# adalca/neurite

Measured on AMD Instinct MI355X. Metric: Mvoxels/sec interpn+Dice on 160^3 x 32-label, higher is better.
Workload: dtype f32

## Files before the change

neurite_amd/csrc/fused_wc.h:

```cpp

#pragma once

#include <type_traits>

#include "dice_reduce.h"
#include "interpn_core.h"

namespace {

#ifndef WC_NST_WARP
#define WC_NST_WARP 3
#endif
#ifndef WC_NST_FUSED
#define WC_NST_FUSED 2
#endif
#ifndef WC_NST_BWD
#define WC_NST_BWD 3
#endif
constexpr int WC_SLOTS = 128;
constexpr int WC_OVF = 16;
constexpr int WC_TRASH_ROW = WC_SLOTS + WC_OVF;
constexpr int WC_ROWS = WC_TRASH_ROW + 1;
constexpr unsigned WC_NOROW = 0x01ffffffu;
constexpr unsigned WC_TAGS_OFF = WC_ROWS * 128;
constexpr unsigned WC_LIST_OFF = WC_TAGS_OFF + 528;
constexpr unsigned WC_BC_OFF = WC_LIST_OFF + 512;
constexpr unsigned WC_WAVE_BYTES = WC_BC_OFF + 128;
constexpr unsigned WC_BLOCK_BYTES = 4 * WC_WAVE_BYTES;
static_assert(WC_LIST_OFF % 16 == 0 && WC_BC_OFF % 16 == 0 && WC_WAVE_BYTES % 16 == 0, "LDS layout");
static_assert((WC_SLOTS + 1) * 4 <= 528 && WC_ROWS <= 256, "LDS layout");
static_assert(2 * WC_BLOCK_BYTES <= 160 * 1024, "two blocks per CU");

typedef __attribute__((address_space(3))) char wc_lds_char;
typedef __attribute__((address_space(3))) nrt_f4 wc_lds_f4;
typedef __attribute__((address_space(3))) volatile nrt_i4 wc_lds_vi4;
typedef __attribute__((address_space(3))) volatile unsigned wc_lds_vu32;
typedef unsigned wc_u3 __attribute__((ext_vector_type(3)));
typedef unsigned wc_u4 __attribute__((ext_vector_type(4)));
typedef float wc_f3 __attribute__((ext_vector_type(3)));

__device__ __forceinline__ void wc_corner(float pv, float mx, int &i0, int &i1, float &w0) {
    const float cl = fminf(fmaxf(pv, 0.0f), mx);
    const float l0 = floorf(cl);
    const float l1 = fminf(nrt_add(l0, 1.0f), mx);
    i0 = (int)l0; i1 = (int)l1;
    w0 = nrt_sub(l1, cl);
}

__device__ __forceinline__ __amdgpu_buffer_rsrc_t wc_rsrc(const void *base, unsigned bytes) {
    const unsigned long long v = (unsigned long long)base;
    const void *u = (const void *)(((unsigned long long)(unsigned)__builtin_amdgcn_readfirstlane((unsigned)(v >> 32)) << 32) |
                                   (unsigned long long)(unsigned)__builtin_amdgcn_readfirstlane((unsigned)v));
    return __builtin_amdgcn_make_buffer_rsrc((void *)u, 0, __builtin_amdgcn_readfirstlane((int)bytes), 0x00020000);
}

struct WcBwd {
    const float *sums, *gdice;
    float eps;
    float *gloc;
};

template <int MODE, bool STORE, bool MM, bool FILL, bool DICE, int BWD = 0>
__device__ __forceinline__ void wc_item(const InterpArgs &a, const TileGeom &tg, const float *__restrict__ fixed, float *__restrict__ fpart,
                                        float *__restrict__ mpart, const XmWork &xw, char *wc_smem, const WcBwd &bw = WcBwd{nullptr, nullptr, 0.0f, nullptr}) {
    constexpr int G = 8, L = 32;
    static_assert(BWD == 0 || (DICE && !STORE && !MM), "the backward form reads a second row per voxel and stores the location gradient only");
    const int b = __builtin_amdgcn_readfirstlane(xw.b);
    const unsigned prow = (unsigned)__builtin_amdgcn_readfirstlane((int)xw.prow), ucol = (unsigned)__builtin_amdgcn_readfirstlane((int)xw.ucol);
    const unsigned RY = 1u << tg.lry, RZ = 1u << tg.lrz;
    const unsigned nRz = (tg.nTz + RZ - 1) / RZ;
    const unsigned reg = ucol / (RY * RZ), wr = ucol % (RY * RZ);
    const unsigned cy = (reg / nRz) * RY + wr / RZ, cz = (reg % nRz) * RZ + wr % RZ;
    const int x0 = __builtin_amdgcn_readfirstlane(xw.x0), y0 = (int)cy << 2, z0 = (int)cz << 3;
    int npass = __builtin_amdgcn_readfirstlane(xw.xlen);
    if (cy >= tg.nTy || cz >= tg.nTz || npass < 0) npass = 0;

    const int lane = threadIdx.x & 63, wave = threadIdx.x >> 6;
    const int g = lane >> 3, p = lane & 7;
    const int dzt = (0x1320 >> ((g & 3) * 4)) & 15;
    const int yy = y0 + 2 * (wave >> 1) + (g >> 2), zz = z0 + 4 * (wave & 1) + dzt;
    const bool yzvalid = (yy < a.O[1]) && (zz < a.O[2]);
    const int yc = min(yy, a.O[1] - 1), zc = min(zz, a.O[2] - 1);
    const unsigned qyz = (unsigned)yc * (unsigned)a.O[2] + (unsigned)zc, qstep = (unsigned)a.O[1] * (unsigned)a.O[2];
    const unsigned SY = (unsigned)a.S[1], SZ = (unsigned)a.S[2];
    const float mxx = (float)(a.S[0] - 1), mxy = (float)(a.S[1] - 1), mxz = (float)(a.S[2] - 1);
    const float fyc = (float)yc, fzc = (float)zc;
    const float ly = (yc == 0) ? 0.0f : ((yc == a.O[1] - 1) ? mxy : nrt_mul(a.delta[1], fyc));
    const float lz = (zc == 0) ? 0.0f : ((zc == a.O[2] - 1) ? mxz : nrt_mul(a.delta[2], fzc));

    const char *volb = (const char *)a.vol + (long long)b * a.vol_bs * 4ll;
    const unsigned long long volbytes = (unsigned long long)a.S[0] * SY * SZ * 128ull;
    const unsigned outbytes = a.nout * 128u;
    const __amdgpu_buffer_rsrc_t vres = wc_rsrc(volb, (unsigned)volbytes);
    const __amdgpu_buffer_rsrc_t lres = wc_rsrc(MODE != NRT_LOC_LINSPACE ? (const char *)(a.loc + (long long)b * a.loc_bs) : volb, a.nout * 12u);
    const __amdgpu_buffer_rsrc_t fres = wc_rsrc(DICE ? (const char *)fixed + (long long)b * a.out_bs * 4ll : volb, outbytes);
    const __amdgpu_buffer_rsrc_t ores = wc_rsrc(STORE ? (const char *)a.out + (long long)b * a.out_bs * 4ll : volb, outbytes);
    const __amdgpu_buffer_rsrc_t gres = wc_rsrc(BWD ? (const char *)(bw.gloc + (long long)b * a.nout * 3) : volb, a.nout * 12u);
    const unsigned gl_lane = (p == 0 && yzvalid) ? qyz * 12u : 0xffffffffu;
    float ca[4] = {0.0f, 0.0f, 0.0f, 0.0f}, cb[4] = {0.0f, 0.0f, 0.0f, 0.0f};
    if (BWD == 1) {
        const float *sm = bw.sums + (long long)b * 3 * L;
#pragma unroll
        for (int k = 0; k < 4; ++k) {
            const int l = p * 4 + k;
            const float num = 2.0f * sm[l] + bw.eps, den = sm[L + l] + sm[2 * L + l] + bw.eps;
            const float gd = bw.gdice[(long long)b * L + l];
            if (den != 0.0f) { ca[k] = 2.0f * gd / den; cb[k] = -2.0f * gd * num / (den * den); }
        }
    }
    const unsigned loc_lane = qyz * 12u, row_lane = (qyz * 8u + (unsigned)p) * 16u;
    const unsigned out_lane = yzvalid ? row_lane : 0xffffffffu;
    const unsigned loc_step = qstep * 12u, row_step = qstep * 128u;
    const unsigned p16 = (unsigned)p * 16u;

    wc_lds_char *wl = (wc_lds_char *)wc_smem + wave * WC_WAVE_BYTES;
    wc_lds_vu32 *tags = (wc_lds_vu32 *)(wl + WC_TAGS_OFF);
    wc_lds_char *lrow = wl + p * 16;
    tags[lane] = ~0u;
    tags[lane + 64] = ~0u;
    const bool cx1 = (p & 4) != 0, cy1 = (p & 2) != 0, cz1 = (p & 1) != 0;

    nrt_f2 stp_l = {0, 0}, stp_h = {0, 0}, stt_l = {0, 0}, stt_h = {0, 0}, spp_l = {0, 0}, spp_h = {0, 0};
    float mnt = INFINITY, mxt = -INFINITY, mnp = INFINITY, mxp = -INFINITY;

    struct Pass {
        float w0x, w0y, w0z;
        unsigned sl[8];
        unsigned lr[4], ld[4];
        unsigned xr[4], xd[4];
        int n;
        int xq;
        float mk[3];
        bool oob;
        nrt_f4 T;
        nrt_f4 F[4], Fx[4];
        float pn[3];
    };
    struct Mg { float w0x, w0y, w0z; bool oob, miss; unsigned rid, slot, t1, t2, mytag; float mk[3]; };
    constexpr int NST = ((BWD ? WC_NST_BWD : (DICE ? WC_NST_FUSED : WC_NST_WARP)) > 2) ? 3 : 2;
    constexpr bool XSH = NST == 3 && DICE;
    Pass A, B, C;
    nrt_f4 FxS[4] = {{0.f, 0.f, 0.f, 0.f}, {0.f, 0.f, 0.f, 0.f}, {0.f, 0.f, 0.f, 0.f}, {0.f, 0.f, 0.f, 0.f}};
    auto reset = [&](Pass &s) {
        s.w0x = s.w0y = s.w0z = 0.f; s.n = 0; s.xq = x0; s.oob = false; s.mk[0] = s.mk[1] = s.mk[2] = 0.f;
        s.T = (nrt_f4){0.f, 0.f, 0.f, 0.f};
#pragma unroll
        for (int i = 0; i < 4; ++i) { s.F[i] = s.Fx[i] = (nrt_f4){0.f, 0.f, 0.f, 0.f}; s.lr[i] = s.xr[i] = WC_NOROW << 7; s.ld[i] = s.xd[i] = WC_TRASH_ROW * 128u; }
#pragma unroll
        for (int i = 0; i < 8; ++i) s.sl[i] = 0;
        s.pn[0] = s.pn[1] = s.pn[2] = 0.f;
    };
    reset(A); reset(B);
    if (NST == 3) reset(C);

    auto fetch_loc = [&](int pass, Pass &s) {
        if (MODE != NRT_LOC_LINSPACE) {
            const wc_u3 v = __builtin_bit_cast(wc_u3, __builtin_amdgcn_raw_buffer_load_b96(lres, loc_lane, (unsigned)(x0 + pass) * loc_step, 0));
            s.pn[0] = __uint_as_float(v[0]); s.pn[1] = __uint_as_float(v[1]); s.pn[2] = __uint_as_float(v[2]);
        }
    };
    auto fetch_row = [&](unsigned rowoff) -> nrt_f4 {
        return __builtin_bit_cast(nrt_f4, __builtin_amdgcn_raw_buffer_load_b128(vres, rowoff | p16, 0, 0));
    };

    auto m1a = [&](int pass, const Pass &s, Mg &m) {
        const int xq = x0 + pass;
        float px, py, pz;
        if (MODE == NRT_LOC_ABSOLUTE) { px = s.pn[0]; py = s.pn[1]; pz = s.pn[2]; }
        else if (MODE == NRT_LOC_SHIFT) { px = nrt_add((float)xq, s.pn[0]); py = nrt_add(fyc, s.pn[1]); pz = nrt_add(fzc, s.pn[2]); }
        else { px = (xq == 0) ? 0.0f : ((xq == a.O[0] - 1) ? mxx : nrt_mul(a.delta[0], (float)xq)); py = ly; pz = lz; }
        int i0x, i1x, i0y, i1y, i0z, i1z;
        wc_corner(px, mxx, i0x, i1x, m.w0x);
        wc_corner(py, mxy, i0y, i1y, m.w0y);
        wc_corner(pz, mxz, i0z, i1z, m.w0z);
        m.oob = FILL ? ((px < 0.0f) || (px > mxx) || (py < 0.0f) || (py > mxy) || (pz < 0.0f) || (pz > mxz)) : false;
        if (BWD) {
            m.mk[0] = (fminf(fmaxf(px, 0.0f), mxx) == px) ? 1.0f : 0.0f;
            m.mk[1] = (fminf(fmaxf(py, 0.0f), mxy) == py) ? 1.0f : 0.0f;
            m.mk[2] = (fminf(fmaxf(pz, 0.0f), mxz) == pz) ? 1.0f : 0.0f;
        }
        const unsigned ix = cx1 ? i1x : i0x, iy = cy1 ? i1y : i0y, iz = cz1 ? i1z : i0z;
        m.rid = nrt_mad24(nrt_mad24(ix, SY, iy), SZ, iz);
        m.slot = ((ix & 3u) << 5) | ((iy & 3u) << 3) | (iz & 7u);
        m.mytag = (m.rid << 6) | (unsigned)lane;
        m.t1 = tags[m.slot];
    };
    auto m1b = [&](Mg &m) {
        m.miss = (m.t1 ^ m.mytag) >= 64u;
        tags[m.miss ? m.slot : (unsigned)WC_SLOTS] = m.mytag;
        m.t2 = tags[m.slot];
    };
    auto m1c = [&](int pass, const Mg &m, Pass &s) {
        const unsigned x2 = m.t2 ^ m.mytag;
        const bool served = x2 < 64u;
        const bool loader = m.miss && x2 == 0u;
        const bool orphan = !served;
        const unsigned long long Ml = __builtin_amdgcn_ballot_w64(loader), Mo = __builtin_amdgcn_ballot_w64(orphan);
        const unsigned long long Mf = Ml | Mo;
        const int no = __builtin_popcountll(Mo);
        int n = __builtin_popcountll(Mf);
        const unsigned ro = __builtin_amdgcn_mbcnt_hi((unsigned)(Mo >> 32), __builtin_amdgcn_mbcnt_lo((unsigned)Mo, 0u));
        const unsigned rf = __builtin_amdgcn_mbcnt_hi((unsigned)(Mf >> 32), __builtin_amdgcn_mbcnt_lo((unsigned)Mf, 0u));
        bool fetcher = loader || orphan;
        unsigned src = orphan ? (unsigned)WC_SLOTS + ro : m.slot;
        unsigned e = fetcher ? rf : (unsigned)n + ((unsigned)lane - rf);
        if (__builtin_expect(no > WC_OVF, 0)) {
            tags[lane] = ~0u;
            tags[lane + 64] = ~0u;
            e = (unsigned)lane; fetcher = true; src = (unsigned)lane; n = 64;
        }
        const unsigned src128 = src * 128u;
        const unsigned tp = ((e & 7u) << 3) | (e >> 3);
        typedef unsigned wc_u2 __attribute__((ext_vector_type(2)));
        *(__attribute__((address_space(3))) volatile wc_u2 *)(wl + WC_LIST_OFF + tp * 8u) =
            (wc_u2){fetcher ? (m.rid << 7) : (WC_NOROW << 7), fetcher ? src128 : (unsigned)WC_TRASH_ROW * 128u};
        ((__attribute__((address_space(3))) volatile unsigned short *)(wl + WC_BC_OFF))[lane] = (unsigned short)src128;
        const nrt_i4 la = *(wc_lds_vi4 *)(wl + WC_LIST_OFF + g * 64), lb = *(wc_lds_vi4 *)(wl + WC_LIST_OFF + g * 64 + 16);
        const nrt_i4 sh = *(wc_lds_vi4 *)(wl + WC_BC_OFF + g * 16);
        s.lr[0] = (unsigned)la[0]; s.ld[0] = (unsigned)la[1]; s.lr[1] = (unsigned)la[2]; s.ld[1] = (unsigned)la[3];
        s.lr[2] = (unsigned)lb[0]; s.ld[2] = (unsigned)lb[1]; s.lr[3] = (unsigned)lb[2]; s.ld[3] = (unsigned)lb[3];
        if (__builtin_expect(n > 32, 0)) {
            const nrt_i4 lc = *(wc_lds_vi4 *)(wl + WC_LIST_OFF + g * 64 + 32), le = *(wc_lds_vi4 *)(wl + WC_LIST_OFF + g * 64 + 48);
            s.xr[0] = (unsigned)lc[0]; s.xd[0] = (unsigned)lc[1]; s.xr[1] = (unsigned)lc[2]; s.xd[1] = (unsigned)lc[3];
            s.xr[2] = (unsigned)le[0]; s.xd[2] = (unsigned)le[1]; s.xr[3] = (unsigned)le[2]; s.xd[3] = (unsigned)le[3];
        }
#pragma unroll
        for (int c = 0; c < 4; ++c) { s.sl[2 * c] = (unsigned)sh[c] & 0xffffu; s.sl[2 * c + 1] = (unsigned)sh[c] >> 16; }
        s.w0x = m.w0x; s.w0y = m.w0y; s.w0z = m.w0z; s.oob = m.oob; s.n = n;
        if (BWD) { s.mk[0] = m.mk[0]; s.mk[1] = m.mk[1]; s.mk[2] = m.mk[2]; }
        s.xq = x0 + pass;
    };
    auto issue = [&](Pass &s) {
#pragma unroll
        for (int i = 0; i < 4; ++i) s.F[i] = fetch_row(s.lr[i]);
        if (!XSH && __builtin_expect(s.n > 32, 0)) {
#pragma unroll
            for (int i = 0; i < 4; ++i) s.Fx[i] = fetch_row(s.xr[i]);
        }
        if (DICE) s.T = __builtin_bit_cast(nrt_f4, __builtin_amdgcn_raw_buffer_load_b128(fres, row_lane, (unsigned)s.xq * row_step, 2));
    };
    auto issue_x = [&](Pass &s) {
        if (XSH && __builtin_expect(s.n > 32, 0)) {
#pragma unroll
            for (int i = 0; i < 4; ++i) FxS[i] = fetch_row(s.xr[i]);
        }
    };
    auto deliver = [&](Pass &s) {
#pragma unroll
        for (int i = 0; i < 4; ++i) *(wc_lds_f4 *)(lrow + s.ld[i]) = s.F[i];
        if (__builtin_expect(s.n > 32, 0)) {
#pragma unroll
            for (int i = 0; i < 4; ++i) *(wc_lds_f4 *)(lrow + s.xd[i]) = XSH ? FxS[i] : s.Fx[i];
        }
    };

    const int last = npass - 1;
    auto step = [&](int pass, Pass &s, Pass &o, Pass &nx, auto masked) {
        constexpr bool MASKED = decltype(masked)::value;
        issue(o);
        __builtin_amdgcn_sched_barrier(0);
        deliver(s);
        nrt_f4 R[8];
#pragma unroll
        for (int corner = 0; corner < 8; ++corner) R[corner] = *(const wc_lds_f4 *)(lrow + s.sl[corner]);
        __builtin_amdgcn_sched_barrier(0);
        Mg m;
        m1a(min(pass + NST, last), s, m);
        __builtin_amdgcn_sched_barrier(0);
        const float w1x = nrt_sub(1.0f, s.w0x), w1y = nrt_sub(1.0f, s.w0y), w1z = nrt_sub(1.0f, s.w0z);
        const nrt_f2 wy2 = {s.w0y, w1y}, wz2 = {s.w0z, w1z};
        const nrt_f2 wxy0 = (nrt_f2){s.w0x, s.w0x} * wy2, wxy1 = (nrt_f2){w1x, w1x} * wy2;
        nrt_f2 wt2[4];
        wt2[0] = (nrt_f2){wxy0[0], wxy0[0]} * wz2;
        wt2[1] = (nrt_f2){wxy0[1], wxy0[1]} * wz2;
        wt2[2] = (nrt_f2){wxy1[0], wxy1[0]} * wz2;
        wt2[3] = (nrt_f2){wxy1[1], wxy1[1]} * wz2;
        nrt_f2 al = {0.0f, 0.0f}, ah = {0.0f, 0.0f};
        constexpr bool BLEND = BWD != 2;
#pragma unroll
        for (int corner = 0; corner < (BLEND ? 4 : 0); ++corner) {
            const float wt = wt2[corner >> 1][corner & 1];
            const nrt_f2 w2 = {wt, wt};
            al = al + w2 * (nrt_f2){R[corner][0], R[corner][1]};
            ah = ah + w2 * (nrt_f2){R[corner][2], R[corner][3]};
        }
        asm volatile("" : "+v"(al), "+v"(ah));
        __builtin_amdgcn_sched_barrier(0);
        m1b(m);
        __builtin_amdgcn_sched_barrier(0);
#pragma unroll
        for (int corner = 4; corner < (BLEND ? 8 : 4); ++corner) {
            const float wt = wt2[corner >> 1][corner & 1];
            const nrt_f2 w2 = {wt, wt};
            al = al + w2 * (nrt_f2){R[corner][0], R[corner][1]};
            ah = ah + w2 * (nrt_f2){R[corner][2], R[corner][3]};
        }
        nrt_f4 acc = {al[0], al[1], ah[0], ah[1]};
        const unsigned xqcur = (unsigned)s.xq;
        const float cw0x = s.w0x, cw0y = s.w0y, cw0z = s.w0z, cmx = s.mk[0], cmy = s.mk[1], cmz = s.mk[2];
        const bool coob = s.oob;
        if (!BWD) {
            if (FILL) {
#pragma unroll
                for (int c = 0; c < 4; ++c) acc[c] = apply_fill(acc[c], s.oob, a.fill_f);
            }
            if (STORE) __builtin_amdgcn_raw_buffer_store_b128(__builtin_bit_cast(wc_u4, acc), ores, out_lane, (unsigned)s.xq * row_step, 2);
        }
        const nrt_f4 Tcur = s.T;
        asm volatile("" : "+v"(acc));
        __builtin_amdgcn_sched_barrier(0);
        m1c(min(pass + NST, last), m, s);
        __builtin_amdgcn_sched_barrier(0);
        if (BWD) {
            nrt_f2 gl2 = {Tcur[0], Tcur[1]}, gh2 = {Tcur[2], Tcur[3]};
            if (BWD == 1) {
                gl2 = __builtin_elementwise_fma((nrt_f2){cb[0], cb[1]}, (nrt_f2){acc[0], acc[1]}, (nrt_f2){ca[0], ca[1]} * gl2);
                gh2 = __builtin_elementwise_fma((nrt_f2){cb[2], cb[3]}, (nrt_f2){acc[2], acc[3]}, (nrt_f2){ca[2], ca[3]} * gh2);
            }
            if (FILL && coob) { gl2 = (nrt_f2){0.0f, 0.0f}; gh2 = gl2; }
            float gacc[3];
            loc_grad_rows(R, gl2, gh2, cw0x, w1x, cw0y, w1y, cw0z, w1z, cmx, cmy, cmz, gacc);
#pragma unroll
            for (int d = 0; d < 3; ++d) {
                float r = gacc[d];
                r += __int_as_float(__builtin_amdgcn_update_dpp(0, __float_as_int(r), 0xB1, 0xF, 0xF, true));
                r += __int_as_float(__builtin_amdgcn_update_dpp(0, __float_as_int(r), 0x4E, 0xF, 0xF, true));
                r += __int_as_float(__builtin_amdgcn_update_dpp(0, __float_as_int(r), 0x141, 0xF, 0xF, true));
                gacc[d] = r;
            }
            __builtin_amdgcn_raw_buffer_store_b96(__builtin_bit_cast(wc_u3, (wc_f3){gacc[0], gacc[1], gacc[2]}), gres, gl_lane, xqcur * loc_step, 0);
        } else if (DICE) {
            nrt_f4 T = Tcur;
            if (MASKED) {
#pragma unroll
                for (int c = 0; c < 4; ++c) { T[c] = yzvalid ? T[c] : 0.0f; acc[c] = yzvalid ? acc[c] : 0.0f; }
            }
            const nrt_f2 pl = {acc[0], acc[1]}, ph = {acc[2], acc[3]}, tl = {T[0], T[1]}, th = {T[2], T[3]};
            stp_l = stp_l + tl * pl; stp_h = stp_h + th * ph;
            stt_l = stt_l + tl * tl; stt_h = stt_h + th * th;
            spp_l = spp_l + pl * pl; spp_h = spp_h + ph * ph;
            if (MM) {
                if (!MASKED || yzvalid) {
#pragma unroll
                    for (int c = 0; c < 4; ++c) {
                        mnt = fminf(mnt, Tcur[c]); mxt = fmaxf(mxt, Tcur[c]);
                        mnp = fminf(mnp, acc[c]); mxp = fmaxf(mxp, acc[c]);
                    }
                }
            }
        }
        if (DICE && !BWD) asm volatile("" : "+v"(stp_l), "+v"(stp_h), "+v"(stt_l), "+v"(stt_h), "+v"(spp_l), "+v"(spp_h));
        else asm volatile("" :: "v"(acc));
        __builtin_amdgcn_sched_barrier(0);
        fetch_loc(min(pass + 2 * NST, last), s);
        issue_x(nx);
        __builtin_amdgcn_sched_barrier(0);
    };
    auto march = [&](auto masked) {
        Mg m;
        if constexpr (NST == 3) {
            fetch_loc(0, A);
            fetch_loc(min(1, last), B);
            fetch_loc(min(2, last), C);
            m1a(0, A, m); m1b(m); m1c(0, m, A);
            issue(A);
            fetch_loc(min(3, last), A);
            m1a(min(1, last), B, m); m1b(m); m1c(min(1, last), m, B);
            issue(B);
            fetch_loc(min(4, last), B);
            m1a(min(2, last), C, m); m1b(m); m1c(min(2, last), m, C);
            fetch_loc(min(5, last), C);
            issue_x(A);
            __builtin_amdgcn_sched_barrier(0);
            int pass = 0;
            for (; pass + 2 < npass; pass += 3) {
                step(pass, A, C, B, masked);
                step(pass + 1, B, A, C, masked);
                step(pass + 2, C, B, A, masked);
            }
            if (pass < npass) step(pass, A, C, B, masked);
            if (pass + 1 < npass) step(pass + 1, B, A, C, masked);
            return;
        }
        fetch_loc(0, A);
        fetch_loc(min(1, last), B);
        m1a(0, A, m); m1b(m); m1c(0, m, A);
        issue(A);
        fetch_loc(min(2, last), A);
        m1a(min(1, last), B, m); m1b(m); m1c(min(1, last), m, B);
        fetch_loc(min(3, last), B);
        __builtin_amdgcn_sched_barrier(0);
        int pass = 0;
        for (; pass + 1 < npass; pass += 2) {
            step(pass, A, B, B, masked);
            step(pass + 1, B, A, A, masked);
        }
        if (pass < npass) step(pass, A, B, B, masked);
    };
    if (npass > 0) {
        if (DICE && !BWD && __builtin_amdgcn_ballot_w64(!yzvalid) != 0ull) march(std::true_type());
        else march(std::false_type());
    }

    if (!DICE || BWD) return;
    nrt_f4 stp = {stp_l[0], stp_l[1], stp_h[0], stp_h[1]}, stt = {stt_l[0], stt_l[1], stt_h[0], stt_h[1]},
           spp = {spp_l[0], spp_l[1], spp_h[0], spp_h[1]};
#pragma unroll
    for (int c = 0; c < 4; ++c) {
        stp[c] = wave_xor_add(stp[c], G);
        stt[c] = wave_xor_add(stt[c], G);
        spp[c] = wave_xor_add(spp[c], G);
    }
    for (int off = 1; off < NRT_WAVE; off <<= 1) {
        mnt = fminf(mnt, __shfl_xor(mnt, off, NRT_WAVE)); mxt = fmaxf(mxt, __shfl_xor(mxt, off, NRT_WAVE));
        mnp = fminf(mnp, __shfl_xor(mnp, off, NRT_WAVE)); mxp = fmaxf(mxp, __shfl_xor(mxp, off, NRT_WAVE));
    }
    __syncthreads();
    float (*red)[3 * L + 4] = (float (*)[3 * L + 4])wc_smem;
    if (lane < G) {
#pragma unroll
        for (int c = 0; c < 4; ++c) {
            red[wave][0 * L + 4 * lane + c] = stp[c];
            red[wave][1 * L + 4 * lane + c] = stt[c];
            red[wave][2 * L + 4 * lane + c] = spp[c];
        }
    }
    if (lane == 0) { red[wave][3 * L + 0] = mnt; red[wave][3 * L + 1] = mxt; red[wave][3 * L + 2] = mnp; red[wave][3 * L + 3] = mxp; }
    __syncthreads();
    const long long pbase = (long long)b * tg.prows + prow;
    for (int i = threadIdx.x; i < 3 * L; i += 256) {
        float s = red[0][i];
#pragma unroll
        for (int w2 = 1; w2 < 4; ++w2) s += red[w2][i];
        fpart[pbase * 3 * L + i] = s;
    }
    if (threadIdx.x < 4) {
        float m = red[0][3 * L + threadIdx.x];
        for (int w2 = 1; w2 < 4; ++w2)
            m = (threadIdx.x & 1) ? fmaxf(m, red[w2][3 * L + threadIdx.x]) : fminf(m, red[w2][3 * L + threadIdx.x]);
        mpart[pbase * 4 + threadIdx.x] = m;
    }
    xmarch_zero_rows(tg, xw, 3 * L, fpart, mpart);
}


template <typename ITEM>
__device__ __forceinline__ void wc_persistent_loop(const TileGeom &tg, int O0, unsigned *__restrict__ queue, ITEM item) {
    __shared__ unsigned s_next[2];
    const unsigned home = blockIdx.x % NRT_NXCD;
    for (;;) {
        __syncthreads();
        if (threadIdx.x == 0) {
            unsigned kk = home, jb = 0xffffffffu;
            for (unsigned t = 0; t < NRT_NXCD; ++t) {
                const unsigned q = (home + t) % NRT_NXCD;
                const unsigned v = atomicAdd(&queue[q * 16u], 1u);
                if (v < tg.items_x) { kk = q; jb = v; break; }
            }
            s_next[0] = kk; s_next[1] = jb;
        }
        __syncthreads();
        const unsigned kk = s_next[0], jb = s_next[1];
        if (jb == 0xffffffffu) break;
        XmWork xw;
        if (!xmarch_work_at(tg, O0, kk, jb, xw)) continue;
        item(xw);
    }
    if (threadIdx.x == 0 && atomicAdd(&queue[NRT_NXCD * 16u], 1u) == gridDim.x - 1) {
        for (unsigned q = 0; q <= NRT_NXCD; ++q) queue[q * 16u] = 0u;
    }
}

template <int MODE, bool STORE, bool MM, bool FILL, bool DICE = true, bool PERSIST = false>
__global__ __launch_bounds__(256, 2) void warp_dice_wc(InterpArgs a, TileGeom tg, const float *__restrict__ fixed,
                                                        float *__restrict__ fpart, float *__restrict__ mpart, unsigned *__restrict__ queue) {
    extern __shared__ __attribute__((aligned(16))) char wc_smem[];
    if (!PERSIST) {
        XmWork xw;
        if (!xmarch_work(tg, a.O[0], xw)) return;
        wc_item<MODE, STORE, MM, FILL, DICE>(a, tg, fixed, fpart, mpart, xw, wc_smem);
        return;
    }
    wc_persistent_loop(tg, a.O[0], queue, [&](const XmWork &xw) { wc_item<MODE, STORE, MM, FILL, DICE>(a, tg, fixed, fpart, mpart, xw, wc_smem); });
}

template <int MODE, bool FILL, int BWD, bool PERSIST>
__global__ __launch_bounds__(256, 2) void warp_dice_wc_bwd(InterpArgs a, TileGeom tg, const float *__restrict__ rows, WcBwd bw,
                                                            unsigned *__restrict__ queue) {
    extern __shared__ __attribute__((aligned(16))) char wc_smem[];
    if (!PERSIST) {
        XmWork xw;
        if (!xmarch_work(tg, a.O[0], xw)) return;
        wc_item<MODE, false, false, FILL, true, BWD>(a, tg, rows, nullptr, nullptr, xw, wc_smem, bw);
        return;
    }
    wc_persistent_loop(tg, a.O[0], queue, [&](const XmWork &xw) { wc_item<MODE, false, false, FILL, true, BWD>(a, tg, rows, nullptr, nullptr, xw, wc_smem, bw); });
}

inline bool wc_persistent(const TileGeom &tg) { return NRT_NXCD * tg.items_x > 2u * (unsigned)nrt_num_cus(); }
static_assert(NRT_RING_GATHER_OFF == 0 && (NRT_NXCD + 1) * 16 <= NRT_RING_CCE_OFF, "the work counters of a launch stay in the gather's words of a slot");

template <int MODE, bool STORE, bool MM, bool FILL>
int launch_wc_inst(const InterpArgs &a, const TileGeom &tg, unsigned nblocks, int batch, const float *fixed, float *fpart, float *mpart,
                   hipStream_t st) {
    const unsigned items = NRT_NXCD * tg.items_x, slots = 2u * (unsigned)nrt_num_cus();
    unsigned *queue = wc_persistent(tg) ? nrt_ring_slot(st) : nullptr;
    if (queue) {
        if (hipFuncSetAttribute((const void *)warp_dice_wc<MODE, STORE, MM, FILL, true, true>, hipFuncAttributeMaxDynamicSharedMemorySize,
                                (int)WC_BLOCK_BYTES) != hipSuccess)
            return NRT_ERR_LAUNCH;
        hipLaunchKernelGGL((warp_dice_wc<MODE, STORE, MM, FILL, true, true>), dim3(nrt_xcd_grid(slots)), dim3(256), WC_BLOCK_BYTES, st, a, tg, fixed,
                           fpart, mpart, queue);
        return NRT_OK;
    }
    if (hipFuncSetAttribute((const void *)warp_dice_wc<MODE, STORE, MM, FILL>, hipFuncAttributeMaxDynamicSharedMemorySize, (int)WC_BLOCK_BYTES) != hipSuccess)
        return NRT_ERR_LAUNCH;
    hipLaunchKernelGGL((warp_dice_wc<MODE, STORE, MM, FILL>), dim3(items), dim3(256), WC_BLOCK_BYTES, st, a, tg, fixed, fpart, mpart,
                       (unsigned *)nullptr);
    (void)nblocks; (void)batch;
    return NRT_OK;
}

template <int MODE, bool FILL>
int launch_wc_fill(const InterpArgs &a, const TileGeom &tg, unsigned nblocks, int batch, bool store, bool minmax, const float *fixed,
                   float *fpart, float *mpart, hipStream_t st) {
    if (store) return minmax ? launch_wc_inst<MODE, true, true, FILL>(a, tg, nblocks, batch, fixed, fpart, mpart, st)
                             : launch_wc_inst<MODE, true, false, FILL>(a, tg, nblocks, batch, fixed, fpart, mpart, st);
    return minmax ? launch_wc_inst<MODE, false, true, FILL>(a, tg, nblocks, batch, fixed, fpart, mpart, st)
                  : launch_wc_inst<MODE, false, false, FILL>(a, tg, nblocks, batch, fixed, fpart, mpart, st);
}

template <int MODE>
int launch_wc_mode(const InterpArgs &a, const TileGeom &tg, unsigned nblocks, int batch, bool store, bool minmax, const float *fixed,
                   float *fpart, float *mpart, hipStream_t st) {
    return a.has_fill ? launch_wc_fill<MODE, true>(a, tg, nblocks, batch, store, minmax, fixed, fpart, mpart, st)
                      : launch_wc_fill<MODE, false>(a, tg, nblocks, batch, store, minmax, fixed, fpart, mpart, st);
}

inline bool wc_applies(const TileGeom &tg, int G, const InterpArgs &a) {
    return tg.x_march && G == 8 && tg.lty == 2 && tg.ltz == 3 && !tg.plane_major &&
           (unsigned long long)a.S[0] * a.S[1] * a.S[2] * 128ull < 0xffffff00ull;
}

inline int launch_wc(const InterpArgs &a, const TileGeom &tg, unsigned nblocks, int batch, int mode, bool store, bool minmax,
                     const float *fixed, float *fpart, float *mpart, hipStream_t st) {
    switch (mode) {
        case NRT_LOC_ABSOLUTE: return launch_wc_mode<NRT_LOC_ABSOLUTE>(a, tg, nblocks, batch, store, minmax, fixed, fpart, mpart, st);
        case NRT_LOC_SHIFT: return launch_wc_mode<NRT_LOC_SHIFT>(a, tg, nblocks, batch, store, minmax, fixed, fpart, mpart, st);
        default: return launch_wc_mode<NRT_LOC_LINSPACE>(a, tg, nblocks, batch, store, minmax, fixed, fpart, mpart, st);
    }
}

template <int MODE, bool FILL>
int launch_wc_interpn_inst(const InterpArgs &a, const TileGeom &tg, hipStream_t st) {
    const unsigned items = NRT_NXCD * tg.items_x, slots = 2u * (unsigned)nrt_num_cus();
    unsigned *queue = (items > slots) ? nrt_ring_slot(st) : nullptr;
    if (queue) {
        if (hipFuncSetAttribute((const void *)warp_dice_wc<MODE, true, false, FILL, false, true>, hipFuncAttributeMaxDynamicSharedMemorySize,
                                (int)WC_BLOCK_BYTES) != hipSuccess)
            return NRT_ERR_LAUNCH;
        hipLaunchKernelGGL((warp_dice_wc<MODE, true, false, FILL, false, true>), dim3(nrt_xcd_grid(slots)), dim3(256), WC_BLOCK_BYTES, st, a, tg,
                           (const float *)nullptr, (float *)nullptr, (float *)nullptr, queue);
        return NRT_OK;
    }
    if (hipFuncSetAttribute((const void *)warp_dice_wc<MODE, true, false, FILL, false>, hipFuncAttributeMaxDynamicSharedMemorySize,
                            (int)WC_BLOCK_BYTES) != hipSuccess)
        return NRT_ERR_LAUNCH;
    hipLaunchKernelGGL((warp_dice_wc<MODE, true, false, FILL, false>), dim3(items), dim3(256), WC_BLOCK_BYTES, st, a, tg, (const float *)nullptr,
                       (float *)nullptr, (float *)nullptr, (unsigned *)nullptr);
    return NRT_OK;
}

template <int MODE, bool FILL, int BWD>
int launch_wc_bwd_inst(const InterpArgs &a, const TileGeom &tg, const float *rows, const WcBwd &bw, hipStream_t st) {
    const unsigned items = NRT_NXCD * tg.items_x, slots = 2u * (unsigned)nrt_num_cus();
    unsigned *queue = (items > slots) ? nrt_ring_slot(st) : nullptr;
    if (queue) {
        if (hipFuncSetAttribute((const void *)warp_dice_wc_bwd<MODE, FILL, BWD, true>, hipFuncAttributeMaxDynamicSharedMemorySize, (int)WC_BLOCK_BYTES) != hipSuccess)
            return NRT_ERR_LAUNCH;
        hipLaunchKernelGGL((warp_dice_wc_bwd<MODE, FILL, BWD, true>), dim3(nrt_xcd_grid(slots)), dim3(256), WC_BLOCK_BYTES, st, a, tg, rows, bw, queue);
        return NRT_OK;
    }
    if (hipFuncSetAttribute((const void *)warp_dice_wc_bwd<MODE, FILL, BWD, false>, hipFuncAttributeMaxDynamicSharedMemorySize, (int)WC_BLOCK_BYTES) != hipSuccess)
        return NRT_ERR_LAUNCH;
    hipLaunchKernelGGL((warp_dice_wc_bwd<MODE, FILL, BWD, false>), dim3(items), dim3(256), WC_BLOCK_BYTES, st, a, tg, rows, bw, (unsigned *)nullptr);
    return NRT_OK;
}

template <int MODE, bool FILL>
int launch_wc_bwd_mode(const InterpArgs &a, const TileGeom &tg, const float *rows, const WcBwd &bw, hipStream_t st) {
    return bw.sums ? launch_wc_bwd_inst<MODE, FILL, 1>(a, tg, rows, bw, st) : launch_wc_bwd_inst<MODE, FILL, 2>(a, tg, rows, bw, st);
}

}

int nrt_wc_bwd_launch(const void *args, int batch, int mode, const float *rows, const float *sums, const float *grad_dice, float eps,
                      float *grad_loc, void *stream) {
    const InterpArgs &a = *(const InterpArgs *)args;
    if (mode != NRT_LOC_ABSOLUTE && mode != NRT_LOC_SHIFT) return NRT_ERR_INVALID_ARG;
    TileGeom tg;
    unsigned nblocks, grid;
    const int t = xmarch_default_tune();
    tile_geometry(a.O, 8, t, t, tg, nblocks);
    xmarch_setup_mixed(a.O, batch, t, tg, grid);
    hipStream_t st = nrt_stream(stream);
    const WcBwd bw = {sums, grad_dice, eps, grad_loc};
    int rc;
    if (mode == NRT_LOC_ABSOLUTE) rc = a.has_fill ? launch_wc_bwd_mode<NRT_LOC_ABSOLUTE, true>(a, tg, rows, bw, st) : launch_wc_bwd_mode<NRT_LOC_ABSOLUTE, false>(a, tg, rows, bw, st);
    else rc = a.has_fill ? launch_wc_bwd_mode<NRT_LOC_SHIFT, true>(a, tg, rows, bw, st) : launch_wc_bwd_mode<NRT_LOC_SHIFT, false>(a, tg, rows, bw, st);
    if (rc != NRT_OK) return rc;
    NRT_CHECK_LAUNCH();
    return NRT_OK;
}

bool nrt_wc_interpn_supported(const void *args, int batch) {
    const InterpArgs &a = *(const InterpArgs *)args;
    if (a.C != 32 || !xmarch_applies(a.O, batch)) return false;
    if ((unsigned long long)a.nout * 128ull >= (1ull << 32)) return false;
    if ((long long)a.S[0] * a.S[1] >= (1 << 24) || a.S[2] >= (1 << 24) || (long long)a.O[0] * a.O[1] >= (1 << 24) || a.O[2] >= (1 << 24)) return false;
    TileGeom tg;
    unsigned nblocks, grid;
    const int t = xmarch_default_tune();
    tile_geometry(a.O, 8, t, t, tg, nblocks);
    xmarch_setup_mixed(a.O, batch, t, tg, grid);
    return wc_applies(tg, 8, a);
}

int nrt_wc_interpn_launch(const void *args, int batch, int mode, void *stream) {
    const InterpArgs &a = *(const InterpArgs *)args;
    TileGeom tg;
    unsigned nblocks, grid;
    const int t = xmarch_default_tune();
    tile_geometry(a.O, 8, t, t, tg, nblocks);
    xmarch_setup_mixed(a.O, batch, t, tg, grid);
    hipStream_t st = nrt_stream(stream);
    int rc;
    switch (mode) {
        case NRT_LOC_ABSOLUTE: rc = a.has_fill ? launch_wc_interpn_inst<NRT_LOC_ABSOLUTE, true>(a, tg, st) : launch_wc_interpn_inst<NRT_LOC_ABSOLUTE, false>(a, tg, st); break;
        case NRT_LOC_SHIFT: rc = a.has_fill ? launch_wc_interpn_inst<NRT_LOC_SHIFT, true>(a, tg, st) : launch_wc_interpn_inst<NRT_LOC_SHIFT, false>(a, tg, st); break;
        default: rc = a.has_fill ? launch_wc_interpn_inst<NRT_LOC_LINSPACE, true>(a, tg, st) : launch_wc_interpn_inst<NRT_LOC_LINSPACE, false>(a, tg, st); break;
    }
    if (rc != NRT_OK) return rc;
    NRT_CHECK_LAUNCH();
    return NRT_OK;
}
```

Measured before the change: 19810.

## Batch sample geometry across passes through per-wave LDS records

```diff
diff --git a/neurite_amd/csrc/fused_wc.h b/neurite_amd/csrc/fused_wc.h
--- a/neurite_amd/csrc/fused_wc.h
+++ b/neurite_amd/csrc/fused_wc.h
@@ -25,11 +25,14 @@
 constexpr unsigned WC_TAGS_OFF = WC_ROWS * 128;
 constexpr unsigned WC_LIST_OFF = WC_TAGS_OFF + 528;
 constexpr unsigned WC_BC_OFF = WC_LIST_OFF + 512;
-constexpr unsigned WC_WAVE_BYTES = WC_BC_OFF + 128;
+constexpr unsigned WC_REC_OFF = WC_BC_OFF + 128;
+constexpr unsigned WC_REC_GROUP = 80;
+constexpr unsigned WC_WAVE_BYTES = WC_REC_OFF + 8 * WC_REC_GROUP;
 constexpr unsigned WC_BLOCK_BYTES = 4 * WC_WAVE_BYTES;
-static_assert(WC_LIST_OFF % 16 == 0 && WC_BC_OFF % 16 == 0 && WC_WAVE_BYTES % 16 == 0, "LDS layout");
+static_assert(WC_LIST_OFF % 16 == 0 && WC_BC_OFF % 16 == 0 && WC_REC_OFF % 16 == 0 && WC_WAVE_BYTES % 16 == 0, "LDS layout");
 static_assert((WC_SLOTS + 1) * 4 <= 528 && WC_ROWS <= 256, "LDS layout");
 static_assert(2 * WC_BLOCK_BYTES <= 160 * 1024, "two blocks per CU");
+static_assert(2 * (WC_BLOCK_BYTES + 8) <= 160 * 1024, "two blocks per CU, the work item's words of a persistent block included");
 
 typedef __attribute__((address_space(3))) char wc_lds_char;
 typedef __attribute__((address_space(3))) nrt_f4 wc_lds_f4;
@@ -45,6 +48,12 @@
     const float l1 = fminf(nrt_add(l0, 1.0f), mx);
     i0 = (int)l0; i1 = (int)l1;
     w0 = nrt_sub(l1, cl);
+}
+
+__device__ __forceinline__ unsigned wc_mad24_su(unsigned a, unsigned b_uniform, unsigned c) {
+    unsigned r;
+    asm("v_mad_u32_u24 %0, %1, %2, %3" : "=v"(r) : "v"(a), "s"(b_uniform), "v"(c));
+    return r;
 }
 
 __device__ __forceinline__ __amdgpu_buffer_rsrc_t wc_rsrc(const void *base, unsigned bytes) {
@@ -134,7 +143,6 @@
         bool oob;
         nrt_f4 T;
         nrt_f4 F[4], Fx[4];
-        float pn[3];
     };
     struct Mg { float w0x, w0y, w0z; bool oob, miss; unsigned rid, slot, t1, t2, mytag; float mk[3]; };
     constexpr int NST = ((BWD ? WC_NST_BWD : (DICE ? WC_NST_FUSED : WC_NST_WARP)) > 2) ? 3 : 2;
@@ -148,40 +156,69 @@
         for (int i = 0; i < 4; ++i) { s.F[i] = s.Fx[i] = (nrt_f4){0.f, 0.f, 0.f, 0.f}; s.lr[i] = s.xr[i] = WC_NOROW << 7; s.ld[i] = s.xd[i] = WC_TRASH_ROW * 128u; }
 #pragma unroll
         for (int i = 0; i < 8; ++i) s.sl[i] = 0;
-        s.pn[0] = s.pn[1] = s.pn[2] = 0.f;
     };
     reset(A); reset(B);
     if (NST == 3) reset(C);
 
-    auto fetch_loc = [&](int pass, Pass &s) {
-        if (MODE != NRT_LOC_LINSPACE) {
-            const wc_u3 v = __builtin_bit_cast(wc_u3, __builtin_amdgcn_raw_buffer_load_b96(lres, loc_lane, (unsigned)(x0 + pass) * loc_step, 0));
-            s.pn[0] = __uint_as_float(v[0]); s.pn[1] = __uint_as_float(v[1]); s.pn[2] = __uint_as_float(v[2]);
-        }
-    };
     auto fetch_row = [&](unsigned rowoff) -> nrt_f4 {
         return __builtin_bit_cast(nrt_f4, __builtin_amdgcn_raw_buffer_load_b128(vres, rowoff | p16, 0, 0));
     };
 
-    auto m1a = [&](int pass, const Pass &s, Mg &m) {
-        const int xq = x0 + pass;
+    constexpr int PER = NST == 2 ? 4 : 3;
+    static_assert(PER * 20 <= WC_REC_GROUP && WC_REC_GROUP % 16 == 0 && PER % NST == 0, "geometry batches");
+    const int last = npass - 1;
+    const int pj = p % PER;
+    wc_lds_char *rec_rd = wl + WC_REC_OFF + g * WC_REC_GROUP;
+    float bl[3] = {0.f, 0.f, 0.f};
+    auto batch_fetch = [&](int kb) {
+        if (MODE != NRT_LOC_LINSPACE) {
+            const unsigned xq = (unsigned)(x0 + min(kb * PER + pj, last));
+            const wc_u3 v = __builtin_bit_cast(wc_u3, __builtin_amdgcn_raw_buffer_load_b96(lres, loc_lane + xq * loc_step, 0, 0));
+            bl[0] = __uint_as_float(v[0]); bl[1] = __uint_as_float(v[1]); bl[2] = __uint_as_float(v[2]);
+        }
+    };
+    auto batch_compute = [&](int kb) {
+        const int xq = x0 + min(kb * PER + pj, last);
         float px, py, pz;
-        if (MODE == NRT_LOC_ABSOLUTE) { px = s.pn[0]; py = s.pn[1]; pz = s.pn[2]; }
-        else if (MODE == NRT_LOC_SHIFT) { px = nrt_add((float)xq, s.pn[0]); py = nrt_add(fyc, s.pn[1]); pz = nrt_add(fzc, s.pn[2]); }
+        if (MODE == NRT_LOC_ABSOLUTE) { px = bl[0]; py = bl[1]; pz = bl[2]; }
+        else if (MODE == NRT_LOC_SHIFT) { px = nrt_add((float)xq, bl[0]); py = nrt_add(fyc, bl[1]); pz = nrt_add(fzc, bl[2]); }
         else { px = (xq == 0) ? 0.0f : ((xq == a.O[0] - 1) ? mxx : nrt_mul(a.delta[0], (float)xq)); py = ly; pz = lz; }
         int i0x, i1x, i0y, i1y, i0z, i1z;
-        wc_corner(px, mxx, i0x, i1x, m.w0x);
-        wc_corner(py, mxy, i0y, i1y, m.w0y);
-        wc_corner(pz, mxz, i0z, i1z, m.w0z);
-        m.oob = FILL ? ((px < 0.0f) || (px > mxx) || (py < 0.0f) || (py > mxy) || (pz < 0.0f) || (pz > mxz)) : false;
+        float w0x, w0y, w0z;
+        wc_corner(px, mxx, i0x, i1x, w0x);
+        wc_corner(py, mxy, i0y, i1y, w0y);
+        wc_corner(pz, mxz, i0z, i1z, w0z);
+        const bool oob = FILL ? ((px < 0.0f) || (px > mxx) || (py < 0.0f) || (py > mxy) || (pz < 0.0f) || (pz > mxz)) : false;
+        unsigned w2 = (((unsigned)i1x & 3u) << 5) | (((unsigned)i1y & 3u) << 3) | ((unsigned)i1z & 7u);
+        w2 |= ((unsigned)(i1x - i0x) << 8) | ((unsigned)(i1y - i0y) << 16) | ((unsigned)(i1z - i0z) << 24) | (oob ? 1u << 25 : 0u);
         if (BWD) {
-            m.mk[0] = (fminf(fmaxf(px, 0.0f), mxx) == px) ? 1.0f : 0.0f;
-            m.mk[1] = (fminf(fmaxf(py, 0.0f), mxy) == py) ? 1.0f : 0.0f;
-            m.mk[2] = (fminf(fmaxf(pz, 0.0f), mxz) == pz) ? 1.0f : 0.0f;
-        }
-        const unsigned ix = cx1 ? i1x : i0x, iy = cy1 ? i1y : i0y, iz = cz1 ? i1z : i0z;
-        m.rid = nrt_mad24(nrt_mad24(ix, SY, iy), SZ, iz);
-        m.slot = ((ix & 3u) << 5) | ((iy & 3u) << 3) | (iz & 7u);
+            w2 |= (fminf(fmaxf(px, 0.0f), mxx) == px) ? 1u << 26 : 0u;
+            w2 |= (fminf(fmaxf(py, 0.0f), mxy) == py) ? 1u << 27 : 0u;
+            w2 |= (fminf(fmaxf(pz, 0.0f), mxz) == pz) ? 1u << 28 : 0u;
+        }
+        const unsigned rid0 = wc_mad24_su(wc_mad24_su(i0x, SY, i0y), SZ, i0z);
+        const unsigned w1 = (rid0 << 7) | (((unsigned)i0x & 3u) << 5) | (((unsigned)i0y & 3u) << 3) | ((unsigned)i0z & 7u);
+        *(wc_lds_vi4 *)(rec_rd + pj * 16) = (nrt_i4){(int)__float_as_uint(w0x), (int)__float_as_uint(w0y), (int)__float_as_uint(w0z), (int)w1};
+        *(wc_lds_vu32 *)(rec_rd + PER * 16 + pj * 4) = w2;
+    };
+    const unsigned cpm = (cx1 ? 0x160u : 0u) | (cy1 ? 0x10018u : 0u) | (cz1 ? 0x1000007u : 0u);
+    const unsigned SYZ = (unsigned)__builtin_amdgcn_readfirstlane((int)(SY * SZ));
+    struct Rec { nrt_i4 r; unsigned w2; };
+    auto rec_read = [&](auto jc, Rec &r) {
+        constexpr int J = decltype(jc)::value;
+        r.r = *(wc_lds_vi4 *)(rec_rd + J * 16);
+        r.w2 = *(wc_lds_vu32 *)(rec_rd + PER * 16 + J * 4);
+    };
+    auto m1a = [&](const Rec &r, Mg &m) {
+        const unsigned w1 = (unsigned)r.r[3], w2 = r.w2;
+        m.w0x = __uint_as_float((unsigned)r.r[0]); m.w0y = __uint_as_float((unsigned)r.r[1]); m.w0z = __uint_as_float((unsigned)r.r[2]);
+        m.oob = FILL ? ((w2 >> 25) & 1u) != 0u : false;
+        if (BWD) {
+            m.mk[0] = (float)((w2 >> 26) & 1u); m.mk[1] = (float)((w2 >> 27) & 1u); m.mk[2] = (float)((w2 >> 28) & 1u);
+        }
+        const unsigned e = w2 & cpm;
+        m.rid = wc_mad24_su((e >> 8) & 1u, SYZ, wc_mad24_su((e >> 16) & 1u, SZ, (w1 >> 7) + (e >> 24)));
+        m.slot = ((w2 & cpm) | (w1 & ~cpm)) & 127u;
         m.mytag = (m.rid << 6) | (unsigned)lane;
         m.t1 = tags[m.slot];
     };
@@ -254,10 +291,12 @@
         }
     };
 
-    const int last = npass - 1;
-    auto step = [&](int pass, Pass &s, Pass &o, Pass &nx, auto masked) {
+    auto step = [&](int pass, Pass &s, Pass &o, Pass &nx, auto masked, auto jc) {
         constexpr bool MASKED = decltype(masked)::value;
+        constexpr bool BATCH = decltype(jc)::value == PER - 1;
         issue(o);
+        Rec rc;
+        rec_read(jc, rc);
         __builtin_amdgcn_sched_barrier(0);
         deliver(s);
         nrt_f4 R[8];
@@ -265,7 +304,7 @@
         for (int corner = 0; corner < 8; ++corner) R[corner] = *(const wc_lds_f4 *)(lrow + s.sl[corner]);
         __builtin_amdgcn_sched_barrier(0);
         Mg m;
-        m1a(min(pass + NST, last), s, m);
+        m1a(rc, m);
         __builtin_amdgcn_sched_barrier(0);
         const float w1x = nrt_sub(1.0f, s.w0x), w1y = nrt_sub(1.0f, s.w0y), w1z = nrt_sub(1.0f, s.w0z);
         const nrt_f2 wy2 = {s.w0y, w1y}, wz2 = {s.w0z, w1z};
@@ -352,50 +391,58 @@
         if (DICE && !BWD) asm volatile("" : "+v"(stp_l), "+v"(stp_h), "+v"(stt_l), "+v"(stt_h), "+v"(spp_l), "+v"(spp_h));
         else asm volatile("" :: "v"(acc));
         __builtin_amdgcn_sched_barrier(0);
-        fetch_loc(min(pass + 2 * NST, last), s);
+        if (BATCH) {
+            const int kb = (pass + NST + 1) / PER;
+            batch_compute(kb);
+            batch_fetch(kb + 1);
+        }
         issue_x(nx);
         __builtin_amdgcn_sched_barrier(0);
     };
     auto march = [&](auto masked) {
         Mg m;
+        Rec rc;
+        const std::integral_constant<int, 0> j0;
+        const std::integral_constant<int, 1> j1;
+        const std::integral_constant<int, 2> j2;
+        const std::integral_constant<int, 3> j3;
+        batch_fetch(0);
+        batch_compute(0);
+        batch_fetch(1);
         if constexpr (NST == 3) {
-            fetch_loc(0, A);
-            fetch_loc(min(1, last), B);
-            fetch_loc(min(2, last), C);
-            m1a(0, A, m); m1b(m); m1c(0, m, A);
+            rec_read(j0, rc); m1a(rc, m); m1b(m); m1c(0, m, A);
             issue(A);
-            fetch_loc(min(3, last), A);
-            m1a(min(1, last), B, m); m1b(m); m1c(min(1, last), m, B);
+            rec_read(j1, rc); m1a(rc, m); m1b(m); m1c(min(1, last), m, B);
             issue(B);
-            fetch_loc(min(4, last), B);
-            m1a(min(2, last), C, m); m1b(m); m1c(min(2, last), m, C);
-            fetch_loc(min(5, last), C);
+            rec_read(j2, rc); m1a(rc, m); m1b(m); m1c(min(2, last), m, C);
+            batch_compute(1);
+            batch_fetch(2);
             issue_x(A);
             __builtin_amdgcn_sched_barrier(0);
             int pass = 0;
             for (; pass + 2 < npass; pass += 3) {
-                step(pass, A, C, B, masked);
-                step(pass + 1, B, A, C, masked);
-                step(pass + 2, C, B, A, masked);
+                step(pass, A, C, B, masked, j0);
+                step(pass + 1, B, A, C, masked, j1);
+                step(pass + 2, C, B, A, masked, j2);
             }
-            if (pass < npass) step(pass, A, C, B, masked);
-            if (pass + 1 < npass) step(pass + 1, B, A, C, masked);
+            if (pass < npass) step(pass, A, C, B, masked, j0);
+            if (pass + 1 < npass) step(pass + 1, B, A, C, masked, j1);
             return;
         }
-        fetch_loc(0, A);
-        fetch_loc(min(1, last), B);
-        m1a(0, A, m); m1b(m); m1c(0, m, A);
+        rec_read(j0, rc); m1a(rc, m); m1b(m); m1c(0, m, A);
         issue(A);
-        fetch_loc(min(2, last), A);
-        m1a(min(1, last), B, m); m1b(m); m1c(min(1, last), m, B);
-        fetch_loc(min(3, last), B);
+        rec_read(j1, rc); m1a(rc, m); m1b(m); m1c(min(1, last), m, B);
         __builtin_amdgcn_sched_barrier(0);
         int pass = 0;
-        for (; pass + 1 < npass; pass += 2) {
-            step(pass, A, B, B, masked);
-            step(pass + 1, B, A, A, masked);
-        }
-        if (pass < npass) step(pass, A, B, B, masked);
+        for (; pass + 3 < npass; pass += 4) {
+            step(pass, A, B, B, masked, j2);
+            step(pass + 1, B, A, A, masked, j3);
+            step(pass + 2, A, B, B, masked, j0);
+            step(pass + 3, B, A, A, masked, j1);
+        }
+        if (pass < npass) step(pass, A, B, B, masked, j2);
+        if (pass + 1 < npass) step(pass + 1, B, A, A, masked, j3);
+        if (pass + 2 < npass) step(pass + 2, A, B, B, masked, j0);
     };
     if (npass > 0) {
         if (DICE && !BWD && __builtin_amdgcn_ballot_w64(!yzvalid) != 0ull) march(std::true_type());
```

Result: no change. 19610 (-1.0%).
